# akanazawa/human_dynamics

Measured on AMD Instinct MI355X. Metric: frames/sec/GPU (ResNet+temporal+SMPL, 224x224); SMPL verts max-abs-err, higher is better.
Workload: dtype f16x3

## Files before the change

### human_dynamics_amd/csrc/stem.hip

```cpp
#include <type_traits>
#include <utility>

#include "stream_kit.h"

namespace {
constexpr int IMG = 224, CONV = 112, POOL = 56, CO = 64;
constexpr int PT = 8;
constexpr int CT = 2 * PT + 1;
constexpr int IP = 2 * CT + 5;
constexpr int IPW = 40;
constexpr int NPIX = CT * CT;
constexpr int MT = (NPIX + 31) / 32;
constexpr int TAPK = 32;
constexpr int WK = 256;

template <typename T> struct StemLds {
    static constexpr int PXB = 4 * (int)sizeof(T);
    static constexpr int PATCH = IP * IPW * PXB;
    static constexpr int WROW = 7 * TAPK * (int)sizeof(T) + 16;
    static constexpr int WTS = CO * WROW;
    static constexpr int CST = MT * 32 * CO * (int)sizeof(T);
    static constexpr int TOTAL = PATCH + (WTS > CST ? WTS : CST);
};

template <typename T> struct StemFrag;
template <> struct StemFrag<float> { typedef f32x4 type; };
template <> struct StemFrag<bf16_t> { typedef bf16x8 type; };

__device__ __forceinline__ f32x16 stem_mma(const f32x4& a, const f32x4& b, f32x16 c) {
#pragma unroll
    for (int j = 0; j < 4; ++j) c = __builtin_amdgcn_mfma_f32_32x32x2f32(a[j], b[j], c, 0, 0, 0);
    return c;
}
__device__ __forceinline__ f32x16 stem_mma(const bf16x8& a, const bf16x8& b, f32x16 c) {
    return __builtin_amdgcn_mfma_f32_32x32x16_bf16(a, b, c, 0, 0, 0);
}

__device__ __forceinline__ void store_rgbx(float* o, float r, float g, float b) {
    *(f32x4*)o = f32x4{r, g, b, 0.f};
}
__device__ __forceinline__ void store_rgbx(bf16_t* o, float r, float g, float b) {
    typedef __attribute__((ext_vector_type(4))) __bf16 bf16x4;
    *(bf16x4*)o = bf16x4{(bf16_t)r, (bf16_t)g, (bf16_t)b, (bf16_t)0.f};
}

template <typename T>
__global__ __launch_bounds__(256) void stem_fused_kernel(const float* __restrict__ img, const T* __restrict__ wts,
                                                         const float* __restrict__ bias,
                                                         const float* __restrict__ pscale,
                                                         const float* __restrict__ pshift, T* __restrict__ out,
                                                         int n_real, const T* __restrict__ w1,
                                                         const float* __restrict__ s1, const float* __restrict__ b1,
                                                         T* __restrict__ out_h1) {
    typedef StemLds<T> LD;
    typedef typename StemFrag<T>::type frag_t;
    constexpr int CPT = (int)sizeof(T);
    extern __shared__ __attribute__((aligned(16))) char smem[];
    char* s_patch = smem;
    char* s_w = smem + LD::PATCH;
    T* s_c = (T*)(smem + LD::PATCH);

    const int tid = threadIdx.x, lane = tid & 63;
    const int wave = __builtin_amdgcn_readfirstlane(tid >> 6);
    const int ty = blockIdx.x / (POOL / PT), tx = blockIdx.x % (POOL / PT);
    const int n = blockIdx.y;
    const int cy0 = 2 * PT * ty, cx0 = 2 * PT * tx;
    const int iy0 = 2 * cy0 - 3, ix0 = 2 * cx0 - 3;

    const float* im = img + (long long)n * IMG * IMG * 3;
    for (int i = tid; i < IP * 11; i += 256) {
        const int py = i / 11, q = i - py * 11;
        const int gy = iy0 + py, gx = ix0 - 1 + 4 * q;
        float f[12];
#pragma unroll
        for (int e = 0; e < 12; ++e) f[e] = 0.f;
        if (n < n_real && (unsigned)gy < (unsigned)IMG && (unsigned)gx < (unsigned)IMG) {
            const f32x4* p = (const f32x4*)(im + (gy * IMG + gx) * 3);
            const f32x4 v0 = p[0], v1 = p[1], v2 = p[2];
#pragma unroll
            for (int e = 0; e < 4; ++e) { f[e] = v0[e]; f[4 + e] = v1[e]; f[8 + e] = v2[e]; }
        }
#pragma unroll
        for (int e = 0; e < 4; ++e) {
            const int px = 4 * q - 1 + e;
            if ((unsigned)px < (unsigned)IPW) {
                T* o = (T*)(s_patch + (py * IPW + px) * LD::PXB);
                store_rgbx(o, f[3 * e], f[3 * e + 1], f[3 * e + 2]);
            }
        }
    }
    constexpr int SLOTS_PER_ROW = 7 * TAPK * (int)sizeof(T) / 16;
    for (int i = tid; i < CO * SLOTS_PER_ROW; i += 256) {
        const int row = i / SLOTS_PER_ROW, sl = i - row * SLOTS_PER_ROW;
        *(u32x4*)(s_w + row * LD::WROW + sl * 16) = *(const u32x4*)((const char*)(wts + (long long)row * WK) + sl * 16);
    }
    __syncthreads();

    const int lr = lane & 31, lh = lane >> 5;
    constexpr int MPW = (MT + 3) / 4;
    f32x16 acc[MPW][2];
#pragma unroll
    for (int i = 0; i < MPW; ++i)
#pragma unroll
        for (int j = 0; j < 2; ++j)
#pragma unroll
            for (int r = 0; r < 16; ++r) acc[i][j][r] = 0.f;
    int abase[MPW];
#pragma unroll
    for (int i = 0; i < MPW; ++i) {
        int p = (wave + 4 * i) * 32 + lr;
        if (p >= NPIX) p = 0;
        const int cy = p / CT, cx = p - cy * CT;
        abase[i] = ((2 * cy) * IPW + 2 * cx) * LD::PXB + lh * 16;
    }
    const int bbase = lr * LD::WROW + lh * 16;
#pragma unroll 1
    for (int ky = 0; ky < 7; ++ky) {
#pragma unroll
        for (int c = 0; c < CPT; ++c) {
            const frag_t b0 = *(const frag_t*)(s_w + bbase + ky * TAPK * (int)sizeof(T) + c * 32);
            const frag_t b1 = *(const frag_t*)(s_w + bbase + 32 * LD::WROW + ky * TAPK * (int)sizeof(T) + c * 32);
#pragma unroll
            for (int i = 0; i < MPW; ++i) {
                if (wave + 4 * i < MT) {
                    const frag_t a = *(const frag_t*)(s_patch + abase[i] + ky * IPW * LD::PXB + c * 32);
                    acc[i][0] = stem_mma(a, b0, acc[i][0]);
                    acc[i][1] = stem_mma(a, b1, acc[i][1]);
                }
            }
        }
    }
    __syncthreads();

#pragma unroll
    for (int i = 0; i < MPW; ++i) {
        if (wave + 4 * i < MT) {
#pragma unroll
            for (int j = 0; j < 2; ++j) {
                const int ch = j * 32 + lr;
                const float bch = bias[ch];
#pragma unroll
                for (int r = 0; r < 16; ++r) {
                    const int p = (wave + 4 * i) * 32 + (r & 3) + 8 * (r >> 2) + 4 * lh;
                    s_c[p * CO + ch] = elem_traits<T>::from_f32(acc[i][j][r] + bch);
                }
            }
        }
    }
    __syncthreads();

    for (int it = tid; it < PT * PT * (CO / 8); it += 256) {
        const int v8 = it & 7, pp = it >> 3;
        const int py = pp / PT, px = pp - py * PT;
        float m[8];
#pragma unroll
        for (int j = 0; j < 8; ++j) m[j] = -3.0e38f;
#pragma unroll
        for (int dy = 0; dy < 3; ++dy) {
            if (cy0 + 2 * py + dy >= CONV) continue;
#pragma unroll
            for (int dx = 0; dx < 3; ++dx) {
                if (cx0 + 2 * px + dx >= CONV) continue;
                float v[8];
                load8(s_c + ((2 * py + dy) * CT + 2 * px + dx) * CO + v8 * 8, v);
#pragma unroll
                for (int j = 0; j < 8; ++j) m[j] = fmaxf(m[j], v[j]);
            }
        }
        float sc[8], sh[8];
        load8(pscale + v8 * 8, sc); load8(pshift + v8 * 8, sh);
#pragma unroll
        for (int j = 0; j < 8; ++j) m[j] = fmaxf(fmaf(m[j], sc[j], sh[j]), 0.f);
        store8(out + (((long long)n * POOL + PT * ty + py) * POOL + PT * tx + px) * CO + v8 * 8, m);
        if constexpr (sizeof(T) == 2) {
            if (out_h1) store8((T*)(s_patch + pp * 128 + ((v8 ^ ((pp >> 1) & 7)) << 4)), m);
        }
    }
    if constexpr (sizeof(T) == 2) {
        if (!out_h1) return;
        __syncthreads();
        const int lr = lane & 31, lh = lane >> 5, fsw = (lr >> 1) & 7;
        const int wn = wave >> 1, wm = wave & 1;
        f32x16 acc1;
#pragma unroll
        for (int r = 0; r < 16; ++r) acc1[r] = 0.f;
#pragma unroll
        for (int kc = 0; kc < 4; ++kc) {
            const bf16x8 a = *(const bf16x8*)(w1 + (long long)(wn * 32 + lr) * 64 + kc * 16 + lh * 8);
            const bf16x8 b = *(const bf16x8*)(s_patch + (wm * 32 + lr) * 128 + (((2 * kc + lh) ^ fsw) << 4));
            acc1 = __builtin_amdgcn_mfma_f32_32x32x16_bf16(a, b, acc1, 0, 0, 0);
        }
        char* s_o = smem + LD::PATCH;
#pragma unroll
        for (int g = 0; g < 4; ++g) {
            const int cl = wn * 32 + 8 * g + 4 * lh;
            const f32x4 s4 = *(const f32x4*)(s1 + cl), b4 = *(const f32x4*)(b1 + cl);
            typedef __attribute__((ext_vector_type(4))) __bf16 bf16x4;
            bf16x4 o;
#pragma unroll
            for (int j = 0; j < 4; ++j) o[j] = (bf16_t)fmaxf(fmaf(acc1[4 * g + j], s4[j], b4[j]), 0.f);
            *(bf16x4*)(s_o + (wm * 32 + lr) * 128 + (((cl >> 3) ^ fsw) << 4) + 8 * lh) = o;
        }
        __syncthreads();
        for (int it = tid; it < PT * PT * (CO / 8); it += 256) {
            const int ps = it & 7, pp = it >> 3, ls = ps ^ ((pp >> 1) & 7);
            const int py = pp / PT, px = pp - py * PT;
            *(u32x4*)(out_h1 + (((long long)n * POOL + PT * ty + py) * POOL + PT * tx + px) * CO + ls * 8) =
                *(const u32x4*)(s_o + pp * 128 + ps * 16);
        }
    }
}
}


namespace {
constexpr int X3_NT = 320, X3_CO = 32;
constexpr int X3_PLANE = IP * IPW * 8;
constexpr int X3_WROW = 7 * TAPK * 2 + 16;
constexpr int X3_WPLANE = X3_CO * X3_WROW;
constexpr int X3_STAGE = MT * 32 * X3_CO * 4;
constexpr int X3_PTILE = PT * PT * 128;
constexpr int X3_LDS0 = 2 * X3_PLANE + (2 * X3_WPLANE > X3_STAGE ? 2 * X3_WPLANE : X3_STAGE);
constexpr int X3_LDS = X3_LDS0 + X3_PTILE;
static_assert(2 * X3_PTILE <= 2 * X3_PLANE + X3_PTILE && 2 * X3_LDS <= 160 * 1024, "two workgroups per CU");

__global__ __launch_bounds__(X3_NT) void stem_fused_split_kernel(const float* __restrict__ img, const bsplit_t* __restrict__ wts,
                                                                 const float* __restrict__ wscale,
                                                                 const float* __restrict__ bias, const float* __restrict__ pscale,
                                                                 const float* __restrict__ pshift, bsplit_t* __restrict__ out,
                                                                 int n_real, const char* __restrict__ w1f, const float* __restrict__ s1,
                                                                 const float* __restrict__ b1, bsplit_t* __restrict__ out_h1) {
    extern __shared__ __attribute__((aligned(16))) char smem[];
    char* s_ph = smem;
    char* s_pl = smem + X3_PLANE;
    char* s_wh = smem + 2 * X3_PLANE;
    char* s_wl = s_wh + X3_WPLANE;
    float* s_c = (float*)(smem + 2 * X3_PLANE);

    const int tid = threadIdx.x, lane = tid & 63;
    const int wave = __builtin_amdgcn_readfirstlane(tid >> 6);
    const int ty = blockIdx.x / (POOL / PT), tx = blockIdx.x % (POOL / PT);
    const int n = blockIdx.y;
    const int cy0 = 2 * PT * ty, cx0 = 2 * PT * tx;
    const int iy0 = 2 * cy0 - 3, ix0 = 2 * cx0 - 3;

    const float* im = img + (long long)n * IMG * IMG * 3;
    float satin = 0.f;
    for (int i = tid; i < IP * 11; i += X3_NT) {
        const int py = i / 11, q = i - py * 11;
        const int gy = iy0 + py, gx = ix0 - 1 + 4 * q;
        float f[12];
#pragma unroll
        for (int e = 0; e < 12; ++e) f[e] = 0.f;
        if (n < n_real && (unsigned)gy < (unsigned)IMG && (unsigned)gx < (unsigned)IMG) {
            const f32x4* p = (const f32x4*)(im + (gy * IMG + gx) * 3);
            const f32x4 v0 = p[0], v1 = p[1], v2 = p[2];
#pragma unroll
            for (int e = 0; e < 4; ++e) { f[e] = v0[e]; f[4 + e] = v1[e]; f[8 + e] = v2[e]; }
#pragma unroll
            for (int e = 0; e < 12; e += 2) satin = sat_acc(satin, f[e], f[e + 1]);
        }
#pragma unroll
        for (int e = 0; e < 4; ++e) {
            const int px = 4 * q - 1 + e;
            if ((unsigned)px < (unsigned)IPW) {
                typedef __attribute__((ext_vector_type(4))) shalf_t shalf4;
                shalf4 h, l;
#pragma unroll
                for (int c = 0; c < 3; ++c) {
                    const float cv = split_clamp(f[3 * e + c]);
                    h[c] = (shalf_t)cv;
                    l[c] = (shalf_t)(cv - (float)h[c]);
                }
                h[3] = (shalf_t)0.f; l[3] = (shalf_t)0.f;
                *(shalf4*)(s_ph + (py * IPW + px) * 8) = h;
                *(shalf4*)(s_pl + (py * IPW + px) * 8) = l;
            }
        }
    }
    split_flag_max(satin);
#pragma unroll 1
    for (int ch0 = 0; ch0 < CO; ch0 += X3_CO) {
    if (ch0) __syncthreads();
    for (int i = tid; i < X3_CO * 28; i += X3_NT) {
        const int row = i / 28, g = i - row * 28;
        const u32x4* src = (const u32x4*)((const char*)wts + (long long)(ch0 + row) * (WK * 4) + g * 32);
        *(u32x4*)(s_wh + row * X3_WROW + g * 16) = src[0];
        *(u32x4*)(s_wl + row * X3_WROW + g * 16) = src[1];
    }
    __syncthreads();

    const int lr = lane & 31, lh = lane >> 5;
    constexpr int MPW = MT / 5;
    static_assert(MPW * 5 == MT, "10 row tiles over 5 waves");
    f32x16 acc[MPW];
#pragma unroll
    for (int i = 0; i < MPW; ++i)
#pragma unroll
        for (int r = 0; r < 16; ++r) acc[i][r] = 0.f;
    int abase[MPW];
#pragma unroll
    for (int i = 0; i < MPW; ++i) {
        int p = (wave + 5 * i) * 32 + lr;
        if (p >= NPIX) p = 0;
        const int cy = p / CT, cx = p - cy * CT;
        abase[i] = ((2 * cy) * IPW + 2 * cx) * 8 + lh * 16;
    }
    const int bbase = lr * X3_WROW + lh * 16;
    const unsigned lds0 = lds_addr(smem);
    const unsigned aw = lds0 + 2 * X3_PLANE + bbase;
    unsigned ap[MPW];
#pragma unroll
    for (int i = 0; i < MPW; ++i) ap[i] = lds0 + abase[i];
    shalf8 fb[2][2], fa[2][MPW][2];
    auto load_step = [&](auto s_c, int set) {
        constexpr int S = decltype(s_c)::value, KY = S >> 1, C = S & 1;
        shalf8& bh = fb[set][0];
        shalf8& bl = fb[set][1];
        bh = lds_rd128<shalf8, KY * 64 + C * 32>(aw);
        bl = lds_rd128<shalf8, X3_WPLANE + KY * 64 + C * 32>(aw);
#pragma unroll
        for (int i = 0; i < MPW; ++i) {
            shalf8& ah = fa[set][i][0];
            shalf8& al = fa[set][i][1];
            const unsigned ad = ap[i];
            ah = lds_rd128<shalf8, KY * IPW * 8 + C * 32>(ad);
            al = lds_rd128<shalf8, X3_PLANE + KY * IPW * 8 + C * 32>(ad);
        }
    };
    auto k_step = [&](auto s_c) {
        constexpr int S = decltype(s_c)::value, CUR = S & 1;
        if constexpr (S + 1 < 14) load_step(ic<(S + 1 < 14 ? S + 1 : 13)>{}, CUR ^ 1);
#pragma unroll
        for (int i = 0; i < MPW; ++i) {
            acc[i] = mfma_split(fa[CUR][i][1], fb[CUR][0], acc[i]);
            acc[i] = mfma_split(fa[CUR][i][0], fb[CUR][1], acc[i]);
            acc[i] = mfma_split(fa[CUR][i][0], fb[CUR][0], acc[i]);
        }
        __builtin_amdgcn_sched_barrier(0);
        wait_lgkm<0>();
        __builtin_amdgcn_sched_barrier(0);
    };
    load_step(ic<0>{}, 0);
    wait_lgkm<0>();
    __builtin_amdgcn_sched_barrier(0);
    auto k_steps = [&](auto... S) { (k_step(S), ...); };
    k_steps(ic<0>{}, ic<1>{}, ic<2>{}, ic<3>{}, ic<4>{}, ic<5>{}, ic<6>{}, ic<7>{}, ic<8>{}, ic<9>{}, ic<10>{}, ic<11>{}, ic<12>{}, ic<13>{});
    __syncthreads();

    {
        const float bch = bias[ch0 + lr];
        const float sch = wscale ? wscale[ch0 + lr] : 1.0f;
#pragma unroll
        for (int i = 0; i < MPW; ++i)
#pragma unroll
            for (int r = 0; r < 16; ++r) {
                const int p = (wave + 5 * i) * 32 + (r & 3) + 8 * (r >> 2) + 4 * lh;
                s_c[p * X3_CO + lr] = stored_value<bsplit_t>(fmaf(acc[i][r], sch, bch));
            }
    }
    __syncthreads();

    for (int it = tid; it < PT * PT * (X3_CO / 8); it += X3_NT) {
        const int v8 = it & 3, pp = it >> 2;
        const int py = pp / PT, px = pp - py * PT;
        float m[8];
#pragma unroll
        for (int j = 0; j < 8; ++j) m[j] = -3.0e38f;
#pragma unroll
        for (int dy = 0; dy < 3; ++dy) {
            if (cy0 + 2 * py + dy >= CONV) continue;
#pragma unroll
            for (int dx = 0; dx < 3; ++dx) {
                if (cx0 + 2 * px + dx >= CONV) continue;
                float v[8];
                load8(s_c + ((2 * py + dy) * CT + 2 * px + dx) * X3_CO + v8 * 8, v);
#pragma unroll
                for (int j = 0; j < 8; ++j) m[j] = fmaxf(m[j], v[j]);
            }
        }
        float sc[8], sh[8];
        load8(pscale + ch0 + v8 * 8, sc); load8(pshift + ch0 + v8 * 8, sh);
#pragma unroll
        for (int j = 0; j < 8; ++j) m[j] = fmaxf(fmaf(m[j], sc[j], sh[j]), 0.f);
        bsplit_t* o = out + (((long long)n * POOL + PT * ty + py) * POOL + PT * tx + px) * CO + ch0 + v8 * 8;
        store8(o, m);
        if (w1f) {
            shalf8 hi, lo;
#pragma unroll
            for (int j = 0; j < 8; ++j) {
                const float cv = split_clamp(m[j]);
                hi[j] = (shalf_t)cv;
                lo[j] = (shalf_t)(cv - (float)hi[j]);
            }
            char* pt = (ch0 ? smem : smem + X3_LDS0) + pp * 128 + ((v8 ^ (pp & 3)) << 5);
            *(shalf8*)pt = hi;
            *(shalf8*)(pt + 16) = lo;
        }
    }
    }
    if (!w1f) return;
    __syncthreads();
    if (wave < 4) {
        const int lr = lane & 31, lh = lane >> 5;
        const int wn = wave >> 1, wm = wave & 1;
        const int p = wm * 32 + lr;
        f32x16 acc1;
#pragma unroll
        for (int r = 0; r < 16; ++r) acc1[r] = 0.f;
#pragma unroll
        for (int kc = 0; kc < 4; ++kc) {
            const shalf8* wp = (const shalf8*)(w1f + ((long long)((wn * 4 + kc) * 64 + lane)) * 32);
            wfrag wf; wf.hi = wp[0]; wf.lo = wp[1];
            const int g = (2 * kc + lh) & 3;
            const char* pt = (kc >= 2 ? smem : smem + X3_LDS0) + p * 128 + ((g ^ (p & 3)) << 5);
            acc1 = mma3(wf, *(const shalf8*)pt, *(const shalf8*)(pt + 16), acc1);
        }
        const int py = p >> 3, px = p & 7;
        bsplit_t* o = out_h1 + (((long long)n * POOL + PT * ty + py) * POOL + PT * tx + px) * CO;
        float satmax = 0.f;
#pragma unroll
        for (int g = 0; g < 4; ++g) {
            const int ch = wn * 32 + 8 * g + 4 * lh;
            const f32x4 s4 = *(const f32x4*)(s1 + ch), b4 = *(const f32x4*)(b1 + ch);
            float v[4];
#pragma unroll
            for (int e = 0; e < 4; ++e) v[e] = fmaf(acc1[4 * g + e], s4[e], b4[e]);
            unsigned h2[2], l2[2];
            split4_mix(v, 0.f, h2, l2, satmax);
            char* og = (char*)o + (wn * 4 + g) * 32 + 8 * lh;
            *(unsigned long long*)og = (unsigned long long)h2[0] | ((unsigned long long)h2[1] << 32);
            *(unsigned long long*)(og + 16) = (unsigned long long)l2[0] | ((unsigned long long)l2[1] << 32);
        }
        split_flag_max(satmax);
    }
}
}

int hmmr_stem_fused(const float* images, int n_real, int n, const void* wts, const float* wscale, const float* bias,
                    const float* pscale, const float* pshift, void* out, int dtype, hipStream_t s,
                    const void* w1, const float* s1, const float* b1, void* out_h1) {
    if (dtype == HMMR_F16X3) {
        static DeviceOnce oncex3;
        return launch_with_lds(stem_fused_split_kernel, oncex3, dim3((POOL / PT) * (POOL / PT), n), dim3(X3_NT), X3_LDS, X3_LDS, s, images,
                               (const bsplit_t*)wts, wscale, bias, pscale, pshift, (bsplit_t*)out, n_real, (const char*)w1, s1, b1,
                               (bsplit_t*)out_h1);
    } else if (dtype == HMMR_BF16) {
        static DeviceOnce once16;
        return launch_with_lds(stem_fused_kernel<bf16_t>, once16, dim3((POOL / PT) * (POOL / PT), n), dim3(256), StemLds<bf16_t>::TOTAL,
                               StemLds<bf16_t>::TOTAL, s, images, (const bf16_t*)wts, bias, pscale, pshift, (bf16_t*)out, n_real,
                               (const bf16_t*)w1, s1, b1, (bf16_t*)out_h1);
    }
    static DeviceOnce once32;
    return launch_with_lds(stem_fused_kernel<float>, once32, dim3((POOL / PT) * (POOL / PT), n), dim3(256), StemLds<float>::TOTAL,
                           StemLds<float>::TOTAL, s, images, (const float*)wts, bias, pscale, pshift, (float*)out, n_real,
                           (const float*)nullptr, (const float*)nullptr, (const float*)nullptr, (float*)nullptr);
}
```

Before: 39570.

## Issue stem patch and weight global loads early into registers before LDS stores

In the bf16 stem kernel, all image-patch and filter global loads are now issued into registers before any LDS stores, so their latencies overlap. In the split stem kernel, patch loads are batched the same way, and the second channel-half's weights are prefetched into registers right after the MFMA loop, then stored to LDS in the next iteration. The channel loop is unrolled and waves_per_eu is pinned to 5. This raises register pressure, which could limit occupancy or cause spills.

```diff
diff --git a/human_dynamics_amd/csrc/stem.hip b/human_dynamics_amd/csrc/stem.hip
--- a/human_dynamics_amd/csrc/stem.hip
+++ b/human_dynamics_amd/csrc/stem.hip
@@ -13,6 +13,10 @@
 constexpr int MT = (NPIX + 31) / 32;
 constexpr int TAPK = 32;
 constexpr int WK = 256;
+
+#ifndef STEM_EARLY_LOADS
+#define STEM_EARLY_LOADS 1
+#endif
 
 template <typename T> struct StemLds {
     static constexpr int PXB = 4 * (int)sizeof(T);
@@ -68,18 +72,7 @@
     const int iy0 = 2 * cy0 - 3, ix0 = 2 * cx0 - 3;
 
     const float* im = img + (long long)n * IMG * IMG * 3;
-    for (int i = tid; i < IP * 11; i += 256) {
-        const int py = i / 11, q = i - py * 11;
-        const int gy = iy0 + py, gx = ix0 - 1 + 4 * q;
-        float f[12];
-#pragma unroll
-        for (int e = 0; e < 12; ++e) f[e] = 0.f;
-        if (n < n_real && (unsigned)gy < (unsigned)IMG && (unsigned)gx < (unsigned)IMG) {
-            const f32x4* p = (const f32x4*)(im + (gy * IMG + gx) * 3);
-            const f32x4 v0 = p[0], v1 = p[1], v2 = p[2];
-#pragma unroll
-            for (int e = 0; e < 4; ++e) { f[e] = v0[e]; f[4 + e] = v1[e]; f[8 + e] = v2[e]; }
-        }
+    auto patch_store = [&](int py, int q, const float (&f)[12]) {
 #pragma unroll
         for (int e = 0; e < 4; ++e) {
             const int px = 4 * q - 1 + e;
@@ -88,11 +81,67 @@
                 store_rgbx(o, f[3 * e], f[3 * e + 1], f[3 * e + 2]);
             }
         }
-    }
+    };
     constexpr int SLOTS_PER_ROW = 7 * TAPK * (int)sizeof(T) / 16;
-    for (int i = tid; i < CO * SLOTS_PER_ROW; i += 256) {
-        const int row = i / SLOTS_PER_ROW, sl = i - row * SLOTS_PER_ROW;
-        *(u32x4*)(s_w + row * LD::WROW + sl * 16) = *(const u32x4*)((const char*)(wts + (long long)row * WK) + sl * 16);
+    if constexpr (!STEM_EARLY_LOADS || sizeof(T) != 2) {
+        for (int i = tid; i < IP * 11; i += 256) {
+            const int py = i / 11, q = i - py * 11;
+            const int gy = iy0 + py, gx = ix0 - 1 + 4 * q;
+            float f[12];
+#pragma unroll
+            for (int e = 0; e < 12; ++e) f[e] = 0.f;
+            if (n < n_real && (unsigned)gy < (unsigned)IMG && (unsigned)gx < (unsigned)IMG) {
+                const f32x4* p = (const f32x4*)(im + (gy * IMG + gx) * 3);
+                const f32x4 v0 = p[0], v1 = p[1], v2 = p[2];
+#pragma unroll
+                for (int e = 0; e < 4; ++e) { f[e] = v0[e]; f[4 + e] = v1[e]; f[8 + e] = v2[e]; }
+            }
+            patch_store(py, q, f);
+        }
+        for (int i = tid; i < CO * SLOTS_PER_ROW; i += 256) {
+            const int row = i / SLOTS_PER_ROW, sl = i - row * SLOTS_PER_ROW;
+            *(u32x4*)(s_w + row * LD::WROW + sl * 16) = *(const u32x4*)((const char*)(wts + (long long)row * WK) + sl * 16);
+        }
+    } else {
+        constexpr int PTRIPS = (IP * 11 + 255) / 256, WTRIPS = CO * SLOTS_PER_ROW / 256;
+        static_assert(WTRIPS * 256 == CO * SLOTS_PER_ROW, "whole filter trips");
+        f32x4 pv[PTRIPS][3];
+        u32x4 wv[WTRIPS];
+#pragma unroll
+        for (int t = 0; t < PTRIPS; ++t) {
+            const int i = tid + t * 256;
+            const int py = i / 11, q = i - py * 11;
+            const int gy = iy0 + py, gx = ix0 - 1 + 4 * q;
+#pragma unroll
+            for (int j = 0; j < 3; ++j) pv[t][j] = f32x4{0.f, 0.f, 0.f, 0.f};
+            if (i < IP * 11 && n < n_real && (unsigned)gy < (unsigned)IMG && (unsigned)gx < (unsigned)IMG) {
+                const f32x4* p = (const f32x4*)(im + (gy * IMG + gx) * 3);
+                pv[t][0] = p[0]; pv[t][1] = p[1]; pv[t][2] = p[2];
+            }
+        }
+#pragma unroll
+        for (int t = 0; t < WTRIPS; ++t) {
+            const int i = tid + t * 256;
+            const int row = i / SLOTS_PER_ROW, sl = i - row * SLOTS_PER_ROW;
+            wv[t] = *(const u32x4*)((const char*)(wts + (long long)row * WK) + sl * 16);
+        }
+#pragma unroll
+        for (int t = 0; t < PTRIPS; ++t) {
+            const int i = tid + t * 256;
+            if (i < IP * 11) {
+                const int py = i / 11, q = i - py * 11;
+                float f[12];
+#pragma unroll
+                for (int e = 0; e < 4; ++e) { f[e] = pv[t][0][e]; f[4 + e] = pv[t][1][e]; f[8 + e] = pv[t][2][e]; }
+                patch_store(py, q, f);
+            }
+        }
+#pragma unroll
+        for (int t = 0; t < WTRIPS; ++t) {
+            const int i = tid + t * 256;
+            const int row = i / SLOTS_PER_ROW, sl = i - row * SLOTS_PER_ROW;
+            *(u32x4*)(s_w + row * LD::WROW + sl * 16) = wv[t];
+        }
     }
     __syncthreads();
 
@@ -223,8 +272,10 @@
 constexpr int X3_LDS0 = 2 * X3_PLANE + (2 * X3_WPLANE > X3_STAGE ? 2 * X3_WPLANE : X3_STAGE);
 constexpr int X3_LDS = X3_LDS0 + X3_PTILE;
 static_assert(2 * X3_PTILE <= 2 * X3_PLANE + X3_PTILE && 2 * X3_LDS <= 160 * 1024, "two workgroups per CU");
-
-__global__ __launch_bounds__(X3_NT) void stem_fused_split_kernel(const float* __restrict__ img, const bsplit_t* __restrict__ wts,
+constexpr int X3_PTRIPS = (IP * 11 + X3_NT - 1) / X3_NT;
+constexpr int X3_WTRIPS = (X3_CO * 28 + X3_NT - 1) / X3_NT;
+
+__global__ __launch_bounds__(X3_NT) __attribute__((amdgpu_waves_per_eu(5, 5))) void stem_fused_split_kernel(const float* __restrict__ img, const bsplit_t* __restrict__ wts,
                                                                  const float* __restrict__ wscale,
                                                                  const float* __restrict__ bias, const float* __restrict__ pscale,
                                                                  const float* __restrict__ pshift, bsplit_t* __restrict__ out,
@@ -246,20 +297,7 @@
 
     const float* im = img + (long long)n * IMG * IMG * 3;
     float satin = 0.f;
-    for (int i = tid; i < IP * 11; i += X3_NT) {
-        const int py = i / 11, q = i - py * 11;
-        const int gy = iy0 + py, gx = ix0 - 1 + 4 * q;
-        float f[12];
-#pragma unroll
-        for (int e = 0; e < 12; ++e) f[e] = 0.f;
-        if (n < n_real && (unsigned)gy < (unsigned)IMG && (unsigned)gx < (unsigned)IMG) {
-            const f32x4* p = (const f32x4*)(im + (gy * IMG + gx) * 3);
-            const f32x4 v0 = p[0], v1 = p[1], v2 = p[2];
-#pragma unroll
-            for (int e = 0; e < 4; ++e) { f[e] = v0[e]; f[4 + e] = v1[e]; f[8 + e] = v2[e]; }
-#pragma unroll
-            for (int e = 0; e < 12; e += 2) satin = sat_acc(satin, f[e], f[e + 1]);
-        }
+    auto patch_store = [&](int py, int q, const float (&f)[12]) {
 #pragma unroll
         for (int e = 0; e < 4; ++e) {
             const int px = 4 * q - 1 + e;
@@ -277,16 +315,93 @@
                 *(shalf4*)(s_pl + (py * IPW + px) * 8) = l;
             }
         }
+    };
+    u32x4 wv[X3_WTRIPS][2];
+    auto wts_load = [&](int ch0) {
+#pragma unroll
+        for (int t = 0; t < X3_WTRIPS; ++t) {
+            const int i = tid + t * X3_NT;
+            if (i < X3_CO * 28) {
+                const int row = i / 28, g = i - row * 28;
+                const u32x4* src = (const u32x4*)((const char*)wts + (long long)(ch0 + row) * (WK * 4) + g * 32);
+                wv[t][0] = src[0];
+                wv[t][1] = src[1];
+            }
+        }
+    };
+    auto wts_store = [&]() {
+#pragma unroll
+        for (int t = 0; t < X3_WTRIPS; ++t) {
+            const int i = tid + t * X3_NT;
+            if (i < X3_CO * 28) {
+                const int row = i / 28, g = i - row * 28;
+                *(u32x4*)(s_wh + row * X3_WROW + g * 16) = wv[t][0];
+                *(u32x4*)(s_wl + row * X3_WROW + g * 16) = wv[t][1];
+            }
+        }
+    };
+    if constexpr (!STEM_EARLY_LOADS) {
+        for (int i = tid; i < IP * 11; i += X3_NT) {
+            const int py = i / 11, q = i - py * 11;
+            const int gy = iy0 + py, gx = ix0 - 1 + 4 * q;
+            float f[12];
+#pragma unroll
+            for (int e = 0; e < 12; ++e) f[e] = 0.f;
+            if (n < n_real && (unsigned)gy < (unsigned)IMG && (unsigned)gx < (unsigned)IMG) {
+                const f32x4* p = (const f32x4*)(im + (gy * IMG + gx) * 3);
+                const f32x4 v0 = p[0], v1 = p[1], v2 = p[2];
+#pragma unroll
+                for (int e = 0; e < 4; ++e) { f[e] = v0[e]; f[4 + e] = v1[e]; f[8 + e] = v2[e]; }
+#pragma unroll
+                for (int e = 0; e < 12; e += 2) satin = sat_acc(satin, f[e], f[e + 1]);
+            }
+            patch_store(py, q, f);
+        }
+    } else {
+        f32x4 pv[X3_PTRIPS][3];
+#pragma unroll
+        for (int t = 0; t < X3_PTRIPS; ++t) {
+            const int i = tid + t * X3_NT;
+            const int py = i / 11, q = i - py * 11;
+            const int gy = iy0 + py, gx = ix0 - 1 + 4 * q;
+#pragma unroll
+            for (int j = 0; j < 3; ++j) pv[t][j] = f32x4{0.f, 0.f, 0.f, 0.f};
+            if (i < IP * 11 && n < n_real && (unsigned)gy < (unsigned)IMG && (unsigned)gx < (unsigned)IMG) {
+                const f32x4* p = (const f32x4*)(im + (gy * IMG + gx) * 3);
+                pv[t][0] = p[0]; pv[t][1] = p[1]; pv[t][2] = p[2];
+            }
+        }
+#pragma unroll
+        for (int t = 0; t < X3_PTRIPS; ++t) {
+            const int i = tid + t * X3_NT;
+            if (i < IP * 11) {
+                const int py = i / 11, q = i - py * 11;
+                float f[12];
+#pragma unroll
+                for (int e = 0; e < 4; ++e) { f[e] = pv[t][0][e]; f[4 + e] = pv[t][1][e]; f[8 + e] = pv[t][2][e]; }
+#pragma unroll
+                for (int e = 0; e < 12; e += 2) satin = sat_acc(satin, f[e], f[e + 1]);
+                patch_store(py, q, f);
+            }
+        }
     }
     split_flag_max(satin);
+#if STEM_EARLY_LOADS
+#pragma unroll
+#else
 #pragma unroll 1
+#endif
     for (int ch0 = 0; ch0 < CO; ch0 += X3_CO) {
     if (ch0) __syncthreads();
-    for (int i = tid; i < X3_CO * 28; i += X3_NT) {
-        const int row = i / 28, g = i - row * 28;
-        const u32x4* src = (const u32x4*)((const char*)wts + (long long)(ch0 + row) * (WK * 4) + g * 32);
-        *(u32x4*)(s_wh + row * X3_WROW + g * 16) = src[0];
-        *(u32x4*)(s_wl + row * X3_WROW + g * 16) = src[1];
+    if (STEM_EARLY_LOADS && ch0) {
+        wts_store();
+    } else {
+        for (int i = tid; i < X3_CO * 28; i += X3_NT) {
+            const int row = i / 28, g = i - row * 28;
+            const u32x4* src = (const u32x4*)((const char*)wts + (long long)(ch0 + row) * (WK * 4) + g * 32);
+            *(u32x4*)(s_wh + row * X3_WROW + g * 16) = src[0];
+            *(u32x4*)(s_wl + row * X3_WROW + g * 16) = src[1];
+        }
     }
     __syncthreads();
 
@@ -346,6 +461,9 @@
     __builtin_amdgcn_sched_barrier(0);
     auto k_steps = [&](auto... S) { (k_step(S), ...); };
     k_steps(ic<0>{}, ic<1>{}, ic<2>{}, ic<3>{}, ic<4>{}, ic<5>{}, ic<6>{}, ic<7>{}, ic<8>{}, ic<9>{}, ic<10>{}, ic<11>{}, ic<12>{}, ic<13>{});
+    if constexpr (STEM_EARLY_LOADS) {
+        if (ch0 + X3_CO < CO) wts_load(ch0 + X3_CO);
+    }
     __syncthreads();
 
     {
```

New measurement: 39720 (median of 6 runs). About the same (+0.4%).
